# johannesu/stereo

Hardware: AMD Instinct MI355X
Metric: TRW-S fusion iterations/sec, 450x375x60 labels (higher is better)
Workload: dtype f64

## Files before the change

stereo_amd/csrc/trws_spec.h:

```cpp
#pragma once
#include <hip/hip_runtime.h>

#include <cstdint>

#include "trws_dev.h"

namespace stereo {
namespace {

constexpr int kSwConsP = 13, kSwPubP = 16, kSwFree = 18, kSwLabel = 20, kSwNode = 22, kSwKinds = 24, kSwPubM = 32;
constexpr int kRsNt = 0, kRsKinds = 1, kRsNmsg = 2, kRsCut = 5, kRsPubKinds = 6, kRsNout = 7, kRsNin = 8, kRsSrc = 9, kRsMd = 13,
              kRsNode = 14, kRsTag = 15;

typedef __attribute__((address_space(3))) int spec_lds_int;
__device__ __forceinline__ int lds_load(const int *w) { return __hip_atomic_load((const spec_lds_int *)w, __ATOMIC_RELAXED, __HIP_MEMORY_SCOPE_WORKGROUP); }
__device__ __forceinline__ void lds_store(int *w, int v) { __hip_atomic_store((spec_lds_int *)w, v, __ATOMIC_RELAXED, __HIP_MEMORY_SCOPE_WORKGROUP); }
#define SPEC_ACQUIRE() __builtin_amdgcn_fence(__ATOMIC_ACQUIRE, "workgroup", "local")
#define SPEC_RELEASE() __builtin_amdgcn_fence(__ATOMIC_RELEASE, "workgroup", "local")

template <int MASK>
__device__ __forceinline__ bool spec_keep_waiting(int &spins, long long &t0, int *abort_word, int32_t *abort_flag, long long spin_ticks) {
  spins = (spins + 1) & MASK;
  if (spins != 0) return true;
  if (lds_load(abort_word) || ld_sc1(abort_flag)) return false;
  const long long now = (long long)wall_clock64();
  if (t0 == 0) { t0 = now | 1; return true; }
  if (now - t0 > 4 * spin_ticks) { lds_store(abort_word, 1); return false; }
  return true;
}
template <bool SLEEP>
__device__ __forceinline__ bool run_wait_i(const int *word, int want, int *abort_word, int32_t *abort_flag, long long spin_ticks) {
  int spins = 0;
  long long t0 = 0;
  while (lds_load(word) < want) {
    if (SLEEP) __builtin_amdgcn_s_sleep(1);
    if (!spec_keep_waiting<SLEEP ? 1023 : 4095>(spins, t0, abort_word, abort_flag, spin_ticks)) return false;
  }
  SPEC_ACQUIRE();
  return true;
}
__device__ __attribute__((noinline)) bool run_wait(const int *word, int want, int *abort_word, int32_t *abort_flag, long long spin_ticks) {
  return run_wait_i<true>(word, want, abort_word, abort_flag, spin_ticks);
}
template <int N>
__device__ __forceinline__ bool run_wait_n(const int *words, int want, int *abort_word, int32_t *abort_flag, long long spin_ticks) {
  static_assert(N == 1 || N == 4, "run_wait_n");
  if (N == 1) return run_wait_i<true>(words, want, abort_word, abort_flag, spin_ticks);
  typedef int spec_v4i __attribute__((ext_vector_type(4)));
  typedef __attribute__((address_space(3))) const volatile spec_v4i spec_lds_v4i;
  int spins = 0;
  long long t0 = 0;
  for (;;) {
    const spec_v4i v = *(spec_lds_v4i *)words;
    if (min(min(v.x, v.y), min(v.z, v.w)) >= want) break;
    if (!spec_keep_waiting<4095>(spins, t0, abort_word, abort_flag, spin_ticks)) return false;
  }
  SPEC_ACQUIRE();
  return true;
}

template <class T>
__device__ __forceinline__ T uniform_value(T v) {
  static_assert(sizeof(T) == 4 || sizeof(T) == 8, "uniform_value");
  if (sizeof(T) == 4) {
    int w;
    __builtin_memcpy(&w, &v, 4);
    w = __builtin_amdgcn_readfirstlane(w);
    __builtin_memcpy(&v, &w, 4);
  } else {
    int w[2];
    __builtin_memcpy(w, &v, 8);
    w[0] = __builtin_amdgcn_readfirstlane(w[0]); w[1] = __builtin_amdgcn_readfirstlane(w[1]);
    __builtin_memcpy(&v, w, 8);
  }
  return v;
}
__device__ __forceinline__ DevParams uniform_params(const DevParams *pp) {
  DevParams q;
#define U(f) q.f = uniform_value(pp->f)
  U(K); U(lambda); U(unary); U(msg); U(pos); U(alpha); U(x); U(done); U(abort_flag); U(spin_ticks); U(n_own); U(N);
  U(desc[0]); U(desc[1]); U(window); U(uniform_step); U(spec_c0[0]); U(spec_c0[1]); U(spec_c1[0]); U(spec_c1[1]);
  U(spec_len); U(spec_nseg); U(spec_max_len); U(spec_rows); U(spec_x); U(spec_undo); U(spec_stat); U(timeline); U(tl_stride); U(debug);
#undef U
  return q;
}

template <int D>
__device__ __forceinline__ int draw_first_ticket(const DevParams &p, int *word) {
  if (threadIdx.x == 0) *word = next_run<D>(p);
  __syncthreads();
  const int run = __builtin_amdgcn_readfirstlane(*word);
  __syncthreads();
  return run;
}

template <class RL, bool PRIMAL, bool UPDATE>
__device__ __attribute__((noinline)) void run_publisher(const DevParams *pp_, int epoch_) {
  extern __shared__ __attribute__((aligned(16))) double spec_lds[];
  const DevParams p = uniform_params(pp_);
  constexpr int R = RL::C * kWave;
  double *rb = spec_lds + RL::kBase;
  int *abort_word = (int *)spec_lds + RL::kAbortInt;
  const int lane = threadIdx.x & (kWave - 1);
  const int epoch = __builtin_amdgcn_readfirstlane(epoch_);
  const int K = p.K;
  int *rw = (int *)(rb + RL::kWords);
  for (int s = 1; s < p.spec_nseg; ++s) {
    const int ps = s & 1;
    if (UPDATE) {
      if (!run_wait_n<RL::C>(rw + kSwPubM + 4 * ps, s, abort_word, p.abort_flag, p.spin_ticks)) return;
      const double *pb = rb + RL::kPub + ps * 2 * R;
      const int kinds = lds_load(rw + kSwKinds + ps);
#pragma unroll
      for (int c = 0; c < RL::C; ++c) {
        const int kk = c * kWave + lane;
        if (kk < K) {
          double a0 = pb[kk], a1 = pb[R + kk];
          if ((p.debug & 16384) && s % 3 == 1 && kk == 0) a0 = __longlong_as_double(__double_as_longlong(a0) ^ 1ll);
          if ((p.debug & 65536) && s % 3 == 1 && (kk & 1)) a0 += 0.375;
#pragma unroll
          for (int k = 0; k < 8; ++k) {
            const int kd = (kinds >> (4 * k)) & 15;
            if (kd) st_sc1(p.spec_rows + ((size_t)s * 8 + k) * K + kk, kd == 8 ? a0 : a1);
          }
        }
      }
    }
    if (PRIMAL) {
      if (!run_wait_i<true>(rw + kSwPubP + ps, s, abort_word, p.abort_flag, p.spin_ticks)) return;
      int label = lds_load(rw + kSwLabel + ps);
      if ((p.debug & 32768) && s % 5 == 2) label = label > 0 ? label - 1 : (K > 1 ? 1 : 0);
      if (lane == 0) st_sc1(p.spec_x + s, label);
    }
    asm volatile("s_waitcnt vmcnt(0)" ::: "memory");
    if (lane == 0) { st_sc1(p.done + p.N + s, epoch); lds_store(rw + kSwFree, s); }
  }
}

template <int C, int WAVES, int VERDICT, bool BACKWARD, bool PRIMAL, bool UPDATE>
__device__ __attribute__((noinline)) int spec_commit(const DevParams *pp_, int epoch_, int p0_, int p1_, int seg_, int compare_, int ctl_off_) {
  extern __shared__ __attribute__((aligned(16))) double spec_lds[];
  const DevParams &p = *pp_;
  const int epoch = epoch_, p0 = p0_, p1 = p1_, seg = seg_, compare = compare_;
  constexpr int D = BACKWARD ? 1 : 0;
  constexpr int DW = TrwsGraph::kDescWords;
  const int32_t *desc = p.desc[D];
  int *ctl = (int *)spec_lds + ctl_off_;
  const int tid = threadIdx.x, lane = tid & (kWave - 1);
  const int wave = __builtin_amdgcn_readfirstlane(tid / kWave);
  const int K = p.K;
  if (compare) {
    if (wave == 0) {
      int differ = 0;
      if (!wait_flag(p, p.N + p.spec_nseg + seg, epoch, -2)) { if (lane == 0) ctl[1] = 1; }
      else {
        const int w = desc[(size_t)p0 * DW + lane];
        const int f = __builtin_amdgcn_readlane(w, 2);
        const int nout = f & 15, ntot = nout + ((f >> 4) & 15);
        for (int j = nout; j < ntot; ++j) {
          if (__builtin_amdgcn_readlane(w, 12 + j) < 0) continue;
          if (UPDATE) {
            const size_t ea = ((size_t)seg * 8 + j) * K, eb = (size_t)__builtin_amdgcn_readlane(w, 4 + j) * K;
            for (int c = 0; c < C; ++c) {
              const int kk = c * kWave + lane, kc = kk < K ? kk : K - 1;
              const double a = ld_sc1(p.spec_rows + ea + kc), b = ld_sc1(p.msg + eb + kc);
              differ |= UNI(__double_as_longlong(a) != __double_as_longlong(b)) ? 1 : 0;
            }
          }
          if (PRIMAL) differ |= ld_sc1(p.spec_x + seg) != ld_sc1(p.x + __builtin_amdgcn_readlane(w, 32 + j)) ? 1 : 0;
        }
      }
      if (lane == 0) ctl[VERDICT] = differ;
    }
    __syncthreads();
    const int differ = __builtin_amdgcn_readfirstlane(ctl[VERDICT]);
    const int gave_up = __builtin_amdgcn_readfirstlane(ctl[1]);
    __syncthreads();
    if (tid == 0) ctl[VERDICT] = 0;
    if (gave_up) { if (tid == 0) st_sc1(p.abort_flag, 1); return 2; }
    if (differ) {
      if (UPDATE) {
        for (int pos = p0 + wave; pos < p1; pos += WAVES) {
          const int w = desc[(size_t)pos * DW + lane];
          const int nout = __builtin_amdgcn_readlane(w, 2) & 15;
          for (int j = 0; j < nout && j < 4; ++j) {
            const size_t em = (size_t)__builtin_amdgcn_readlane(w, 4 + j) * K, eu = ((size_t)(seg * p.spec_max_len + (pos - p0)) * 4 + j) * K;
            for (int c = 0; c < C; ++c) {
              const int kk = c * kWave + lane;
              if (kk < K) st_sc1(p.msg + em + kk, ld_sc1(p.spec_undo + eu + kk));
            }
          }
        }
        asm volatile("s_waitcnt vmcnt(0)" ::: "memory");
        __builtin_amdgcn_fence(__ATOMIC_ACQ_REL, "agent");
      }
      if (tid == 0) { ctl[3] = 1; if (p.spec_stat) atomicAdd(p.spec_stat, 1ull); }
      __syncthreads();
      return 1;
    }
  }
  if (wave == 0) {
    if (seg + 1 < p.spec_nseg && lane == 0) st_sc1(p.done + p.N + p.spec_nseg + seg + 1, epoch);
    for (int pos = p0 + lane; pos < p1; pos += kWave) st_sc1(p.done + desc[(size_t)pos * DW + 1], epoch);
    if (lane == 0 && p.spec_stat) atomicAdd(p.spec_stat + 1, 1ull);
  }
  return 0;
}

template <class RL, bool BACKWARD, bool PRIMAL, bool UPDATE>
__device__ __attribute__((noinline)) void chain_runner(const DevParams *pp_, int epoch_) {
  extern __shared__ __attribute__((aligned(16))) double spec_lds[];
  const DevParams &p = *pp_;
  const int epoch = epoch_;
  constexpr int R = RL::C * kWave, M = RL::kMsgWaves, D = BACKWARD ? 1 : 0;
  double *rb = spec_lds + RL::kBase;
  const int tid = threadIdx.x;
  const int wave = __builtin_amdgcn_readfirstlane(tid / kWave);
  const int c0 = p.spec_c0[D], c1 = p.spec_c1[D];
  int *rw = (int *)(rb + RL::kWords);
  if (tid < 64) rw[tid] = 0;
  if (tid < RL::kSlots) ((int *)(rb + tid * RL::kSlotDoubles + RL::kSc))[kRsTag] = 0;
  if (tid < 32 * RL::kTabs) {
    const int t = tid >> 5, e = tid & 31;
    rb[RL::kTab + t * (R + 32) + (e < 16 ? e : R + e)] = __builtin_huge_val();
  }
  RL::prepare(p, rb, tid);
  if (p.timeline && tid == 0) p.timeline[((size_t)2 * p.tl_stride + D) * 2] = wall_clock64();
  __syncthreads();
  const unsigned long long trole0 = wall_clock64();
  if (wave < M) { if (UPDATE) { __builtin_amdgcn_s_setprio(3); RL::template messages<BACKWARD>(pp_, wave); __builtin_amdgcn_s_setprio(0); } }
  else if (wave == M) { if (PRIMAL) { __builtin_amdgcn_s_setprio(3); RL::template labels<BACKWARD>(pp_); __builtin_amdgcn_s_setprio(0); } }
  else if (wave < M + 1 + RL::kLoaders) RL::template loader<BACKWARD, PRIMAL, UPDATE>(pp_, epoch, wave - M - 1);
  else if (wave == M + 1 + RL::kLoaders) run_publisher<RL, PRIMAL, UPDATE>(pp_, epoch);
  if (p.timeline && p.spec_stat && (tid & (kWave - 1)) == 0 && (wave == 0 || wave == M || wave == M + RL::kLoaders || wave == M + 1 + RL::kLoaders))
    p.spec_stat[8 + 4 * D + (wave == 0 ? 0 : wave == M ? 1 : wave == M + RL::kLoaders ? 2 : 3)] = wall_clock64() - trole0;
  __syncthreads();
  if (RL::kOverlay && lds_load((int *)spec_lds + RL::kAbortInt) && tid == 0) st_sc1(p.abort_flag, 1);
  if (p.timeline && tid == 0) p.timeline[((size_t)2 * p.tl_stride + D) * 2 + 1] = wall_clock64();
  if (p.spec_stat && tid == 0) atomicAdd(p.spec_stat + 2, (unsigned long long)(c1 - c0));
  if (RL::kOverlay) __syncthreads();
}

constexpr int kRunSlots = 10;
constexpr int kRunLoaders = 8;
constexpr int kRunRowP = 0, kRunRowS = 64, kRunRowM = 256, kRunRowTH = 384, kRunRowOUT = 448, kRunSc = 704;
constexpr int kRunSlotDoubles = kRunSc + 16;
constexpr int kRunTab = kRunSlots * kRunSlotDoubles;
constexpr int kRunPub = kRunTab + 96;
constexpr int kRunWords = kRunPub + 256;
constexpr int kRunDoubles = kRunWords + 32;
constexpr int kRunDummy = 32;
constexpr int kRwConsM = 12;
constexpr int kRunBase = kPipeLdsDoubles, kRunAbortInt = 2 * kPipeCtlOff + 1;

#define RLI(v, i) __builtin_amdgcn_readlane((v), (i))

struct RunNodeM {
  int sw;
  double sd, P, S0, S1, S2, M0, M1;
};
__device__ __forceinline__ void run_request_m(const double *sl, int lane, RunNodeM &n) {
  n.sw = ((const int *)(sl + kRunSc))[lane & 15];
  asm volatile("" ::: "memory");
  n.sd = sl[kRunSc + 8 + (lane & 7)];
  n.P = sl[kRunRowP + lane]; n.S0 = sl[kRunRowS + lane]; n.S1 = sl[kRunRowS + 64 + lane]; n.S2 = sl[kRunRowS + 128 + lane];
  n.M0 = sl[kRunRowM + lane]; n.M1 = sl[kRunRowM + 64 + lane];
}
struct RunArgsM {
  int K, window, c0, c1;
  double lambda, step;
  int32_t *abort_flag;
  long long spin_ticks;
  unsigned long long *stat;
};

template <bool BACKWARD, int G>
__device__ __forceinline__ bool run_visit_m(const RunArgsM &a, double *rb, int *rw, double *tabl, int *cons_word, int lane, bool act, int i, int &slot_off,
                                            RunNodeM &cur, RunNodeM &nxt, double &A0, double &A1, double (&ad)[4 * G], double &alpha_have,
                                            int *abort_word) {
  const double inf = __builtin_huge_val();
  if (__builtin_amdgcn_readlane(cur.sw, kRsTag) != i + 1) {
    const long long t0_ = (long long)wall_clock64();
    if (!__builtin_amdgcn_readfirstlane((int)run_wait((const int *)(rb + slot_off + kRunSc) + kRsTag, i + 1, abort_word, a.abort_flag, a.spin_ticks))) return false;
    run_request_m(rb + slot_off, lane, cur);
    if (a.stat && lane == 0) { atomicAdd(a.stat + 3 + 2 * (BACKWARD ? 1 : 0), 1ull); atomicAdd(a.stat + 4 + 2 * (BACKWARD ? 1 : 0), (unsigned long long)((long long)wall_clock64() - t0_)); }
  }
  const int sw = cur.sw;
  const int key = __builtin_amdgcn_readlane(sw, kRsKinds), nmsg = __builtin_amdgcn_readlane(sw, kRsNmsg), cut = __builtin_amdgcn_readlane(sw, kRsCut);
  double Di = cur.P;
  if (key == 0x20098) { Di += A0; Di += A1; }
  else if (key == 0x30908) { Di += A0; Di += cur.S0; Di += A1; }
  else if (key == 0x30098) { Di += A0; Di += A1; Di += cur.S0; }
  else if (key == 0x41908) { Di += A0; Di += cur.S0; Di += A1; Di += cur.S1; }
  else {
    const int nt = key >> 16;
    for (int t = 0; t < nt; ++t) {
      const int kd = (key >> (4 * t)) & 15;
      if (kd == 8) Di += A0; else if (kd == 9) Di += A1; else if (kd == 0) Di += cur.S0; else if (kd == 1) Di += cur.S1; else Di += cur.S2;
    }
  }
  if (BACKWARD) Di -= wave_min_dpp(act ? Di : inf);
  const double sd = cur.sd, mold0 = cur.M0, mold1 = cur.M1;
  const double gamma = readlane_f64(sd, 2);
  lds_store(cons_word, i + 1 - a.c0);
  slot_off += kRunSlotDoubles;
  if (slot_off == kRunSlots * kRunSlotDoubles) slot_off = 0;
  if (i + 1 < a.c1) run_request_m(rb + slot_off, lane, nxt);
  double R0 = 0, R1 = 0;
  for (int m = 0; m < nmsg; ++m) {
    const double alpha = readlane_f64(sd, m);
    const double h = gamma * Di - (m == 0 ? mold0 : mold1);
    double out = 0;
    if (alpha != 0) {
      *tabl = h;
      if (__builtin_expect(alpha != alpha_have, 0)) {
        asm volatile("" ::: "memory");
#pragma unroll
        for (int d = 0; d < 4 * G; ++d) ad[d] = alpha * ((double)(d + 1) * a.step);
        alpha_have = alpha;
      }
      const double hmin = wave_min_dpp(h);
      const double vtrunc = hmin + alpha * a.lambda;
      __builtin_amdgcn_fence(__ATOMIC_RELEASE, "wavefront");
      __builtin_amdgcn_wave_barrier();
      double lo[4 * G], hi[4 * G];
#pragma unroll
      for (int d = 0; d < 4 * G; ++d) { lo[d] = tabl[-(d + 1)]; hi[d] = tabl[d + 1]; }
      double ma = h, mb = vtrunc;
#pragma unroll
      for (int d = 0; d < 4 * G; ++d) { ma = min_raw(ma, lo[d] + ad[d]); mb = min_raw(mb, hi[d] + ad[d]); }
      __builtin_amdgcn_fence(__ATOMIC_ACQUIRE, "wavefront");
      __builtin_amdgcn_wave_barrier();
      out = min_raw(ma, mb) - hmin;
    }
    if (m == 0) R0 = out; else R1 = out;
  }
  A0 = R0; A1 = nmsg == 2 ? R1 : R0;
  if (cut) {
    const int ps = cut & 1;
    if (__builtin_amdgcn_readfirstlane(lds_load(rw + kSwFree)) < cut - 2 &&
        !__builtin_amdgcn_readfirstlane((int)run_wait(rw + kSwFree, cut - 2, abort_word, a.abort_flag, a.spin_ticks))) return false;
    double *pb = rb + kRunPub + ps * 128;
    pb[lane] = A0; pb[64 + lane] = A1;
    if (lane == 0) lds_store(rw + kSwKinds + ps, __builtin_amdgcn_readlane(sw, kRsPubKinds));
    SPEC_RELEASE();
    if (lane == 0) lds_store(rw + kSwPubM + 4 * ps, cut);
  }
  return true;
}

template <bool BACKWARD, int G>
__device__ __forceinline__ void run_messages_g(const RunArgsM &a, double *rb, int lane, int *abort_word) {
  const bool act = lane < a.K;
  int *rw = (int *)(rb + kRunWords);
  double *tabl = rb + kRunTab + 16 + lane;
  int *cons_word = lane == 0 ? rw + kRwConsM : (int *)(rb + kRunDoubles) + lane;
  double ad[4 * G];
#pragma unroll
  for (int d = 0; d < 4 * G; ++d) ad[d] = 0;
  double alpha_have = 0;
  double A0 = 0, A1 = 0;
  RunNodeM na, nb;
  run_request_m(rb, lane, na);
  nb = na;
  int slot_off = 0;
  for (int i = a.c0; i < a.c1; i += 2) {
    if (!run_visit_m<BACKWARD, G>(a, rb, rw, tabl, cons_word, lane, act, i, slot_off, na, nb, A0, A1, ad, alpha_have, abort_word)) return;
    if (i + 1 < a.c1 && !run_visit_m<BACKWARD, G>(a, rb, rw, tabl, cons_word, lane, act, i + 1, slot_off, nb, na, A0, A1, ad, alpha_have, abort_word)) return;
  }
}

template <bool BACKWARD>
__device__ __attribute__((noinline)) void run_messages(const DevParams *pp) {
  extern __shared__ __attribute__((aligned(16))) double run_lds[];
  constexpr int D = BACKWARD ? 1 : 0;
  RunArgsM a;
  a.K = uniform_value(pp->K); a.window = uniform_value(pp->window); a.c0 = uniform_value(pp->spec_c0[D]); a.c1 = uniform_value(pp->spec_c1[D]);
  a.lambda = uniform_value(pp->lambda); a.step = uniform_value(pp->uniform_step);
  a.abort_flag = uniform_value(pp->abort_flag); a.spin_ticks = uniform_value(pp->spin_ticks); a.stat = uniform_value(pp->spec_stat);
  double *rb = run_lds + kRunBase;
  int *abort_word = (int *)run_lds + kRunAbortInt;
  const int lane = threadIdx.x & (kWave - 1);
  if (a.window <= 4) run_messages_g<BACKWARD, 1>(a, rb, lane, abort_word);
  else run_messages_g<BACKWARD, 2>(a, rb, lane, abort_word);
}

struct RunNodeP {
  int sw;
  double sd, TH, O0, O1, O2, O3;
};
__device__ __forceinline__ void run_request_p(const double *sl, int lane, RunNodeP &n) {
  n.sw = ((const int *)(sl + kRunSc))[lane & 15];
  asm volatile("" ::: "memory");
  n.sd = sl[kRunSc + 8 + (lane & 7)];
  n.TH = sl[kRunRowTH + lane];
  n.O0 = sl[kRunRowOUT + lane]; n.O1 = sl[kRunRowOUT + 64 + lane]; n.O2 = sl[kRunRowOUT + 128 + lane]; n.O3 = sl[kRunRowOUT + 192 + lane];
}
template <bool BACKWARD>
__device__ __attribute__((noinline)) void run_labels(const DevParams *pp_) {
  extern __shared__ __attribute__((aligned(16))) double run_lds[];
  const DevParams p = uniform_params(pp_);
  double *rb = run_lds + kRunBase;
  int *abort_word = (int *)run_lds + kRunAbortInt;
  const int lane = threadIdx.x & (kWave - 1);
  const int c0 = p.spec_c0[BACKWARD ? 1 : 0], c1 = p.spec_c1[BACKWARD ? 1 : 0];
  const double inf = __builtin_huge_val();
  const int K = p.K;
  const bool act = lane < K;
  int *rw = (int *)(rb + kRunWords);
  const double posk = act ? p.pos[lane] : 0.0;
  const double lambda = p.lambda;
  int xprev = 0;
  RunNodeP cur, nxt;
  run_request_p(rb, lane, cur);
  nxt = cur;
  for (int i = c0; i < c1; ++i) {
    const double *sl = rb + ((i - c0) % kRunSlots) * kRunSlotDoubles;
    if (RLI(cur.sw, kRsTag) != i + 1) {
      if (!run_wait_i<true>((const int *)(sl + kRunSc) + kRsTag, i + 1, abort_word, p.abort_flag, p.spin_ticks)) return;
      run_request_p(sl, lane, cur);
    }
    const int sw = cur.sw;
    const double sd = cur.sd;
    const int nout = RLI(sw, kRsNout), nin = RLI(sw, kRsNin), md = RLI(sw, kRsMd), cut = RLI(sw, kRsCut);
    double db = act ? cur.TH : 0.0;
    const double o0 = cur.O0, o1 = cur.O1, o2 = cur.O2, o3 = cur.O3;
    if (lane == 0) lds_store(rw + kSwConsP, i + 1 - c0);
    if (i + 1 < c1) run_request_p(rb + ((i + 1 - c0) % kRunSlots) * kRunSlotDoubles, lane, nxt);
#pragma unroll
    for (int k = 0; k < 4; ++k) {
      if (k < nin) {
        const int src = RLI(sw, kRsSrc + k);
        const int ks = src < 0 ? xprev : src;
        const double pks = readlane_f64(posk, ks);
        const double d = ((md >> k) & 1) == 0 ? pks - posk : posk - pks;
        db += readlane_f64(sd, 3 + k) * min_raw(fabs(d), lambda);
      }
    }
    double di = db;
    if (nout > 0) di += o0;
    if (nout > 1) di += o1;
    if (nout > 2) di += o2;
    if (nout > 3) di += o3;
    const double dim = act ? di : inf;
    const double vbest = wave_min_dpp(dim);
    xprev = __builtin_ctzll(__builtin_amdgcn_ballot_w64(dim == vbest));
    if (cut) {
      const int ps = cut & 1;
      if (!run_wait_i<true>(rw + kSwFree, cut - 2, abort_word, p.abort_flag, p.spin_ticks)) return;
      if (lane == 0) { rw[kSwLabel + ps] = xprev; rw[kSwNode + ps] = RLI(sw, kRsNode); }
      SPEC_RELEASE();
      if (lane == 0) lds_store(rw + kSwPubP + ps, cut);
    }
    cur = nxt;
  }
}

template <bool BACKWARD, bool PRIMAL, bool UPDATE>
__device__ __attribute__((noinline)) void run_loader(const DevParams *pp_, int epoch_, int lw_) {
  extern __shared__ __attribute__((aligned(16))) double run_lds[];
  const DevParams p = uniform_params(pp_);
  double *rb = run_lds + kRunBase;
  int *abort_word = (int *)run_lds + kRunAbortInt;
  const int lane = threadIdx.x & (kWave - 1);
  const int epoch = __builtin_amdgcn_readfirstlane(epoch_), lw = __builtin_amdgcn_readfirstlane(lw_);
  constexpr int D = BACKWARD ? 1 : 0;
  const int c0 = p.spec_c0[D], c1 = p.spec_c1[D];
  constexpr int DW = TrwsGraph::kDescWords;
  const int32_t *desc = p.desc[D];
  const int K = p.K;
  const int lk = lane < K ? lane : K - 1;
  int *rw = (int *)(rb + kRunWords);
  const int L = p.spec_len, nseg = p.spec_nseg;
  int w2 = 0, wn2 = 0;
  if (c0 + lw < c1) { w2 = desc[(size_t)(c0 + lw) * DW + lane]; wn2 = c0 + lw + 1 < c1 ? desc[(size_t)(c0 + lw + 1) * DW + lane] : 0; }
  for (int i = c0 + lw; i < c1; i += kRunLoaders) {
    const int w = w2, wn = wn2;
    if (i + kRunLoaders < c1) {
      w2 = desc[(size_t)(i + kRunLoaders) * DW + lane];
      wn2 = i + kRunLoaders + 1 < c1 ? desc[(size_t)(i + kRunLoaders + 1) * DW + lane] : 0;
    }
    const int f = RLI(w, 2), fn = RLI(wn, 2);
    const int nout = f & 15, nin = (f >> 4) & 15, ndep = (f >> 8) & 15, md = (f >> 16) & 255, ntot = nout + nin;
    const int noutn = fn & 15, ntotn = noutn + ((fn >> 4) & 15);
    const int j8 = lane & 7;
    const int slw = __shfl(w, 12 + j8, kWave), sln = __shfl(wn, 12 + j8, kWave);
    const int fr = i > c0 ? (int)(__builtin_amdgcn_ballot_w64(lane < 8 && lane >= nout && lane < ntot && slw >= 0) & 255ull) : 0;
    const int frn = i + 1 < c1 ? (int)(__builtin_amdgcn_ballot_w64(lane < 8 && lane >= noutn && lane < ntotn && sln >= 0) & 255ull) : 0;
    const int kfirst = fr ? __builtin_ctz(fr) : ntot;
    int s0 = -1, s1 = -1;
    {
      int rest = frn;
      while (rest) {
        const int k = __builtin_ctz(rest);
        rest &= rest - 1;
        const int s = __builtin_amdgcn_readlane(wn, 12 + k);
        if (s0 < 0 || s0 == s) s0 = s; else s1 = s;
      }
    }
    int p0s = -1;
    if (fr) p0s = __builtin_amdgcn_readlane(w, 12 + kfirst);
    int kinds = 0, nt = 0, nstaged = 0, stage_of[4] = {-1, -1, -1, -1};
    for (int k = kfirst; k < ntot; ++k) {
      int kd;
      if ((fr >> k) & 1) kd = __builtin_amdgcn_readlane(w, 12 + k) == p0s ? 8 : 9;
      else { kd = nstaged; if (nstaged < 4) stage_of[nstaged] = k; ++nstaged; }
      kinds |= kd << (4 * nt);
      ++nt;
    }
    int cut = 0, pubkinds = 0;
    if (i + 1 < c1 && (i + 1 - c0) % L == 0 && (i + 1 - c0) / L < nseg) {
      cut = (i + 1 - c0) / L;
      for (int k = noutn; k < ntotn; ++k)
        if ((frn >> k) & 1) pubkinds |= (__builtin_amdgcn_readlane(wn, 12 + k) == s0 ? 8 : 9) << (4 * k);
    }
    const int fm = RLI(w, kDescFetch) & 255;
    const double *ua = p.unary + (size_t)((unsigned long long)(unsigned)RLI(w, 0) * (unsigned long long)(unsigned)K) + lk;
    const double theta = *ua;
    const double av = p.alpha[__shfl(w, 4 + j8, kWave)];
    double r[8];
#pragma unroll
    for (int k = 0; k < 8; ++k) {
      r[k] = 0;
      if (k < nout) r[k] = *(p.msg + (size_t)((unsigned long long)(unsigned)RLI(w, 4 + k) * (unsigned long long)(unsigned)K) + lk);
    }
    if (ndep > 0) wait_for_dependencies_w(p, ndep, __shfl(w, 20 + (lane & 3), kWave), RLI(w, 1), epoch, lane, abort_word);
    if (lds_load(abort_word)) return;
    int src = -1;
#pragma unroll
    for (int k = 0; k < 8; ++k) {
      if (k >= nout && k < ntot && ((fm >> k) & 1) && !((fr >> k) & 1)) {
        if (UPDATE) r[k] = ld_sc1(p.msg + (size_t)((unsigned long long)(unsigned)RLI(w, 4 + k) * (unsigned long long)(unsigned)K) + lk);
        if (PRIMAL) { const int xv = ld_sc1(p.x + RLI(w, 32 + k)); if (lane == k - nout) src = xv; }
      }
    }
    double *sl = rb + ((i - c0) % kRunSlots) * kRunSlotDoubles;
    if (UPDATE && !run_wait_i<true>(rw + kRwConsM, i - c0 - kRunSlots + 1, abort_word, p.abort_flag, p.spin_ticks)) return;
    if (PRIMAL && !run_wait_i<true>(rw + kSwConsP, i - c0 - kRunSlots + 1, abort_word, p.abort_flag, p.spin_ticks)) return;
    if (UPDATE) {
      double P = theta;
#pragma unroll
      for (int k = 0; k < 8; ++k)
        if (k < kfirst) P += r[k];
      sl[kRunRowP + lane] = P;
#pragma unroll
      for (int k = 0; k < 8; ++k) {
        if (stage_of[0] == k) sl[kRunRowS + lane] = r[k];
        if (stage_of[1] == k) sl[kRunRowS + 64 + lane] = r[k];
        if (stage_of[2] == k) sl[kRunRowS + 128 + lane] = r[k];
      }
#pragma unroll
      for (int k = 0; k < 4; ++k) {
        if (s0 == k) sl[kRunRowM + lane] = lane < K ? r[k] : -__builtin_huge_val();
        if (s1 == k) sl[kRunRowM + 64 + lane] = lane < K ? r[k] : -__builtin_huge_val();
      }
    }
    if (PRIMAL) {
      sl[kRunRowTH + lane] = theta;
#pragma unroll
      for (int k = 0; k < 4; ++k)
        if (k < nout) sl[kRunRowOUT + k * 64 + lane] = r[k];
    }
    int nmsg = s0 < 0 ? 0 : 1;
    if (UPDATE && s1 >= 0) {
      bool same = RLI(__double2hiint(av), s0) == RLI(__double2hiint(av), s1) && RLI(__double2loint(av), s0) == RLI(__double2loint(av), s1);
#pragma unroll
      for (int a = 0; a < 4; ++a)
#pragma unroll
        for (int b = 0; b < 4; ++b)
          if (a != b && s0 == a && s1 == b) same = same && !UNI(lane < K && __double_as_longlong(r[a]) != __double_as_longlong(r[b]));
      nmsg = same ? 1 : 2;
    }
    {
      int word = 0;
      word = lane == kRsNt ? nt : lane == kRsKinds ? (kinds | (nt << 16)) : lane == kRsNmsg ? nmsg : lane == kRsCut ? cut
           : lane == kRsPubKinds ? pubkinds : lane == kRsNout ? nout : lane == kRsNin ? nin : lane == kRsMd ? (md >> nout) : lane == kRsNode ? RLI(w, 0) : 0;
      const int srck = __shfl(src, lane - kRsSrc, kWave);
      if (lane >= kRsSrc && lane < kRsSrc + 4) word = srck;
      if (lane < kRsTag) ((int *)(sl + kRunSc))[lane] = word;
      const double a0 = readlane_f64(av, s0 < 0 ? 0 : s0), a1 = readlane_f64(av, s1 < 0 ? (s0 < 0 ? 0 : s0) : s1);
      const double ain = __shfl(av, nout + (lane - 3 < 0 ? 0 : lane - 3), kWave);
      const double g = (double)1 / (double)(nout > nin ? nout : nin > 0 ? nin : 1);
      if (lane < 8) sl[kRunSc + 8 + lane] = lane == 0 ? a0 : lane == 1 ? a1 : lane == 2 ? g : ain;
    }
    SPEC_RELEASE();
    if (lane == 0) lds_store((int *)(sl + kRunSc) + kRsTag, i + 1);
  }
}

struct PipeRunner {
  static constexpr int C = 1, kBase = kRunBase, kAbortInt = kRunAbortInt, kSlots = kRunSlots, kSlotDoubles = kRunSlotDoubles,
                       kSc = kRunSc, kTab = kRunTab, kTabs = 1, kPub = kRunPub, kWords = kRunWords, kMsgWaves = 1, kLoaders = kRunLoaders;
  static constexpr bool kOverlay = false;
  static __device__ __forceinline__ void prepare(const DevParams &, double *, int) {}
  template <bool BACKWARD>
  static __device__ __forceinline__ void messages(const DevParams *pp, int) { run_messages<BACKWARD>(pp); }
  template <bool BACKWARD>
  static __device__ __forceinline__ void labels(const DevParams *pp) { run_labels<BACKWARD>(pp); }
  template <bool BACKWARD, bool PRIMAL, bool UPDATE>
  static __device__ __forceinline__ void loader(const DevParams *pp, int epoch, int lw) { run_loader<BACKWARD, PRIMAL, UPDATE>(pp, epoch, lw); }
};

#undef RLI

}
}
```

Before: 129.1.

## Restructure label wave loop and reschedule message min-convolution in speculative TRW-S

The label-decoding wave is rewritten to match the message wave: a 2-way unrolled ping-pong node pipeline with an incrementally advanced slot offset instead of a modulo, per-lane consumption words, and a fast-path check before waiting on the free word. The message wave gains fast paths for the dominant per-direction kind keys and hoists alpha*lambda into a cached value. The wave min reduction is moved after the neighbour table loads, separated by scheduling barriers, so LDS latency overlaps the DPP reduction. LDS base pointers are pinned to 32-bit scalar address-space values so the compiler can use cheaper addressing. The risk is added ordering subtlety from the extra acquire fence and the changed reduction order.

```diff
diff --git a/stereo_amd/csrc/trws_spec.h b/stereo_amd/csrc/trws_spec.h
--- a/stereo_amd/csrc/trws_spec.h
+++ b/stereo_amd/csrc/trws_spec.h
@@ -15,6 +15,12 @@
 typedef __attribute__((address_space(3))) int spec_lds_int;
 __device__ __forceinline__ int lds_load(const int *w) { return __hip_atomic_load((const spec_lds_int *)w, __ATOMIC_RELAXED, __HIP_MEMORY_SCOPE_WORKGROUP); }
 __device__ __forceinline__ void lds_store(int *w, int v) { __hip_atomic_store((spec_lds_int *)w, v, __ATOMIC_RELAXED, __HIP_MEMORY_SCOPE_WORKGROUP); }
+typedef __attribute__((address_space(3))) double spec_lds_double;
+__device__ __forceinline__ double *pinned_lds(double *dyn) {
+  unsigned off = (unsigned)(size_t)(spec_lds_double *)dyn;
+  asm volatile("" : "+s"(off));
+  return (double *)(spec_lds_double *)(size_t)off;
+}
 #define SPEC_ACQUIRE() __builtin_amdgcn_fence(__ATOMIC_ACQUIRE, "workgroup", "local")
 #define SPEC_RELEASE() __builtin_amdgcn_fence(__ATOMIC_RELEASE, "workgroup", "local")
 
@@ -276,7 +282,7 @@
 
 template <bool BACKWARD, int G>
 __device__ __forceinline__ bool run_visit_m(const RunArgsM &a, double *rb, int *rw, double *tabl, int *cons_word, int lane, bool act, int i, int &slot_off,
-                                            RunNodeM &cur, RunNodeM &nxt, double &A0, double &A1, double (&ad)[4 * G], double &alpha_have,
+                                            RunNodeM &cur, RunNodeM &nxt, double &A0, double &A1, double (&ad)[4 * G], double &alpha_have, double &al,
                                             int *abort_word) {
   const double inf = __builtin_huge_val();
   if (__builtin_amdgcn_readlane(cur.sw, kRsTag) != i + 1) {
@@ -288,7 +294,13 @@
   const int sw = cur.sw;
   const int key = __builtin_amdgcn_readlane(sw, kRsKinds), nmsg = __builtin_amdgcn_readlane(sw, kRsNmsg), cut = __builtin_amdgcn_readlane(sw, kRsCut);
   double Di = cur.P;
-  if (key == 0x20098) { Di += A0; Di += A1; }
+  int key_first = key;
+  asm volatile("" : "+s"(key_first));
+  const bool between = BACKWARD && key_first == 0x30908;
+  if (BACKWARD) key_first ^= between ? 0x30908 ^ 0x30098 : 0;
+  if (!BACKWARD && __builtin_expect(key_first == 0x20098, 1)) { Di += A0; Di += A1; }
+  else if (BACKWARD && __builtin_expect(key_first == 0x30098, 1)) { Di += A0; Di += between ? cur.S0 : A1; Di += between ? A1 : cur.S0; }
+  else if (key == 0x20098) { Di += A0; Di += A1; }
   else if (key == 0x30908) { Di += A0; Di += cur.S0; Di += A1; }
   else if (key == 0x30098) { Di += A0; Di += A1; Di += cur.S0; }
   else if (key == 0x41908) { Di += A0; Di += cur.S0; Di += A1; Di += cur.S1; }
@@ -317,21 +329,24 @@
         asm volatile("" ::: "memory");
 #pragma unroll
         for (int d = 0; d < 4 * G; ++d) ad[d] = alpha * ((double)(d + 1) * a.step);
+        al = alpha * a.lambda;
         alpha_have = alpha;
       }
-      const double hmin = wave_min_dpp(h);
-      const double vtrunc = hmin + alpha * a.lambda;
       __builtin_amdgcn_fence(__ATOMIC_RELEASE, "wavefront");
       __builtin_amdgcn_wave_barrier();
       double lo[4 * G], hi[4 * G];
 #pragma unroll
       for (int d = 0; d < 4 * G; ++d) { lo[d] = tabl[-(d + 1)]; hi[d] = tabl[d + 1]; }
-      double ma = h, mb = vtrunc;
-#pragma unroll
-      for (int d = 0; d < 4 * G; ++d) { ma = min_raw(ma, lo[d] + ad[d]); mb = min_raw(mb, hi[d] + ad[d]); }
+      __builtin_amdgcn_sched_barrier(0);
+      const double hmin = wave_min_dpp(h);
+      __builtin_amdgcn_sched_barrier(0);
+      const double vtrunc = hmin + al;
+      double ma = h, mb = hi[0] + ad[0];
+#pragma unroll
+      for (int d = 0; d < 4 * G; ++d) { ma = min_raw(ma, lo[d] + ad[d]); if (d > 0) mb = min_raw(mb, hi[d] + ad[d]); }
       __builtin_amdgcn_fence(__ATOMIC_ACQUIRE, "wavefront");
       __builtin_amdgcn_wave_barrier();
-      out = min_raw(ma, mb) - hmin;
+      out = min_raw(min_raw(ma, mb), vtrunc) - hmin;
     }
     if (m == 0) R0 = out; else R1 = out;
   }
@@ -359,14 +374,15 @@
 #pragma unroll
   for (int d = 0; d < 4 * G; ++d) ad[d] = 0;
   double alpha_have = 0;
+  double al = 0;
   double A0 = 0, A1 = 0;
   RunNodeM na, nb;
   run_request_m(rb, lane, na);
   nb = na;
   int slot_off = 0;
   for (int i = a.c0; i < a.c1; i += 2) {
-    if (!run_visit_m<BACKWARD, G>(a, rb, rw, tabl, cons_word, lane, act, i, slot_off, na, nb, A0, A1, ad, alpha_have, abort_word)) return;
-    if (i + 1 < a.c1 && !run_visit_m<BACKWARD, G>(a, rb, rw, tabl, cons_word, lane, act, i + 1, slot_off, nb, na, A0, A1, ad, alpha_have, abort_word)) return;
+    if (!run_visit_m<BACKWARD, G>(a, rb, rw, tabl, cons_word, lane, act, i, slot_off, na, nb, A0, A1, ad, alpha_have, al, abort_word)) return;
+    if (i + 1 < a.c1 && !run_visit_m<BACKWARD, G>(a, rb, rw, tabl, cons_word, lane, act, i + 1, slot_off, nb, na, A0, A1, ad, alpha_have, al, abort_word)) return;
   }
 }
 
@@ -378,8 +394,9 @@
   a.K = uniform_value(pp->K); a.window = uniform_value(pp->window); a.c0 = uniform_value(pp->spec_c0[D]); a.c1 = uniform_value(pp->spec_c1[D]);
   a.lambda = uniform_value(pp->lambda); a.step = uniform_value(pp->uniform_step);
   a.abort_flag = uniform_value(pp->abort_flag); a.spin_ticks = uniform_value(pp->spin_ticks); a.stat = uniform_value(pp->spec_stat);
-  double *rb = run_lds + kRunBase;
-  int *abort_word = (int *)run_lds + kRunAbortInt;
+  double *lds0 = pinned_lds(run_lds);
+  double *rb = lds0 + kRunBase;
+  int *abort_word = (int *)lds0 + kRunAbortInt;
   const int lane = threadIdx.x & (kWave - 1);
   if (a.window <= 4) run_messages_g<BACKWARD, 1>(a, rb, lane, abort_word);
   else run_messages_g<BACKWARD, 2>(a, rb, lane, abort_word);
@@ -396,63 +413,82 @@
   n.TH = sl[kRunRowTH + lane];
   n.O0 = sl[kRunRowOUT + lane]; n.O1 = sl[kRunRowOUT + 64 + lane]; n.O2 = sl[kRunRowOUT + 128 + lane]; n.O3 = sl[kRunRowOUT + 192 + lane];
 }
+struct RunArgsP {
+  int c0, c1;
+  double lambda;
+  int32_t *abort_flag;
+  long long spin_ticks;
+};
+__device__ __forceinline__ bool run_visit_p(const RunArgsP &a, double *rb, int *rw, int *cons_word, int lane, bool act, double posk, int i, int &slot_off,
+                                            RunNodeP &cur, RunNodeP &nxt, int &xprev, int *abort_word) {
+  const double inf = __builtin_huge_val();
+  if (RLI(cur.sw, kRsTag) != i + 1) {
+    if (!__builtin_amdgcn_readfirstlane((int)run_wait((const int *)(rb + slot_off + kRunSc) + kRsTag, i + 1, abort_word, a.abort_flag, a.spin_ticks))) return false;
+    run_request_p(rb + slot_off, lane, cur);
+  }
+  const int sw = cur.sw;
+  const double sd = cur.sd;
+  const int nout = RLI(sw, kRsNout), nin = RLI(sw, kRsNin), md = RLI(sw, kRsMd), cut = RLI(sw, kRsCut);
+  double db = act ? cur.TH : 0.0;
+  const double o0 = cur.O0, o1 = cur.O1, o2 = cur.O2, o3 = cur.O3;
+  lds_store(cons_word, i + 1 - a.c0);
+  slot_off += kRunSlotDoubles;
+  if (slot_off == kRunSlots * kRunSlotDoubles) slot_off = 0;
+  if (i + 1 < a.c1) run_request_p(rb + slot_off, lane, nxt);
+#pragma unroll
+  for (int k = 0; k < 4; ++k) {
+    if (k < nin) {
+      const int src = RLI(sw, kRsSrc + k);
+      const int ks = src < 0 ? xprev : src;
+      const double pks = readlane_f64(posk, ks);
+      const double d = ((md >> k) & 1) == 0 ? pks - posk : posk - pks;
+      db += readlane_f64(sd, 3 + k) * min_raw(fabs(d), a.lambda);
+    }
+  }
+  double di = db;
+  if (nout > 0) di += o0;
+  if (nout > 1) di += o1;
+  if (nout > 2) di += o2;
+  if (nout > 3) di += o3;
+  const double dim = act ? di : inf;
+  const double vbest = wave_min_dpp(dim);
+  xprev = __builtin_ctzll(__builtin_amdgcn_ballot_w64(dim == vbest));
+  if (cut) {
+    const int ps = cut & 1;
+    if (__builtin_amdgcn_readfirstlane(lds_load(rw + kSwFree)) < cut - 2 &&
+        !__builtin_amdgcn_readfirstlane((int)run_wait(rw + kSwFree, cut - 2, abort_word, a.abort_flag, a.spin_ticks))) return false;
+    SPEC_ACQUIRE();
+    if (lane == 0) { rw[kSwLabel + ps] = xprev; rw[kSwNode + ps] = RLI(sw, kRsNode); }
+    SPEC_RELEASE();
+    if (lane == 0) lds_store(rw + kSwPubP + ps, cut);
+  }
+  return true;
+}
 template <bool BACKWARD>
-__device__ __attribute__((noinline)) void run_labels(const DevParams *pp_) {
+__device__ __attribute__((noinline)) void run_labels(const DevParams *pp) {
   extern __shared__ __attribute__((aligned(16))) double run_lds[];
-  const DevParams p = uniform_params(pp_);
-  double *rb = run_lds + kRunBase;
-  int *abort_word = (int *)run_lds + kRunAbortInt;
+  constexpr int D = BACKWARD ? 1 : 0;
+  RunArgsP a;
+  a.c0 = uniform_value(pp->spec_c0[D]); a.c1 = uniform_value(pp->spec_c1[D]); a.lambda = uniform_value(pp->lambda);
+  a.abort_flag = uniform_value(pp->abort_flag); a.spin_ticks = uniform_value(pp->spin_ticks);
+  const int K = uniform_value(pp->K);
+  const double *pos = uniform_value(pp->pos);
+  double *lds0 = pinned_lds(run_lds);
+  double *rb = lds0 + kRunBase;
+  int *abort_word = (int *)lds0 + kRunAbortInt;
   const int lane = threadIdx.x & (kWave - 1);
-  const int c0 = p.spec_c0[BACKWARD ? 1 : 0], c1 = p.spec_c1[BACKWARD ? 1 : 0];
-  const double inf = __builtin_huge_val();
-  const int K = p.K;
   const bool act = lane < K;
   int *rw = (int *)(rb + kRunWords);
-  const double posk = act ? p.pos[lane] : 0.0;
-  const double lambda = p.lambda;
+  int *cons_word = lane == 0 ? rw + kSwConsP : (int *)(rb + kRunDoubles) + lane;
+  const double posk = act ? pos[lane] : 0.0;
   int xprev = 0;
-  RunNodeP cur, nxt;
-  run_request_p(rb, lane, cur);
-  nxt = cur;
-  for (int i = c0; i < c1; ++i) {
-    const double *sl = rb + ((i - c0) % kRunSlots) * kRunSlotDoubles;
-    if (RLI(cur.sw, kRsTag) != i + 1) {
-      if (!run_wait_i<true>((const int *)(sl + kRunSc) + kRsTag, i + 1, abort_word, p.abort_flag, p.spin_ticks)) return;
-      run_request_p(sl, lane, cur);
-    }
-    const int sw = cur.sw;
-    const double sd = cur.sd;
-    const int nout = RLI(sw, kRsNout), nin = RLI(sw, kRsNin), md = RLI(sw, kRsMd), cut = RLI(sw, kRsCut);
-    double db = act ? cur.TH : 0.0;
-    const double o0 = cur.O0, o1 = cur.O1, o2 = cur.O2, o3 = cur.O3;
-    if (lane == 0) lds_store(rw + kSwConsP, i + 1 - c0);
-    if (i + 1 < c1) run_request_p(rb + ((i + 1 - c0) % kRunSlots) * kRunSlotDoubles, lane, nxt);
-#pragma unroll
-    for (int k = 0; k < 4; ++k) {
-      if (k < nin) {
-        const int src = RLI(sw, kRsSrc + k);
-        const int ks = src < 0 ? xprev : src;
-        const double pks = readlane_f64(posk, ks);
-        const double d = ((md >> k) & 1) == 0 ? pks - posk : posk - pks;
-        db += readlane_f64(sd, 3 + k) * min_raw(fabs(d), lambda);
-      }
-    }
-    double di = db;
-    if (nout > 0) di += o0;
-    if (nout > 1) di += o1;
-    if (nout > 2) di += o2;
-    if (nout > 3) di += o3;
-    const double dim = act ? di : inf;
-    const double vbest = wave_min_dpp(dim);
-    xprev = __builtin_ctzll(__builtin_amdgcn_ballot_w64(dim == vbest));
-    if (cut) {
-      const int ps = cut & 1;
-      if (!run_wait_i<true>(rw + kSwFree, cut - 2, abort_word, p.abort_flag, p.spin_ticks)) return;
-      if (lane == 0) { rw[kSwLabel + ps] = xprev; rw[kSwNode + ps] = RLI(sw, kRsNode); }
-      SPEC_RELEASE();
-      if (lane == 0) lds_store(rw + kSwPubP + ps, cut);
-    }
-    cur = nxt;
+  RunNodeP na, nb;
+  run_request_p(rb, lane, na);
+  nb = na;
+  int slot_off = 0;
+  for (int i = a.c0; i < a.c1; i += 2) {
+    if (!run_visit_p(a, rb, rw, cons_word, lane, act, posk, i, slot_off, na, nb, xprev, abort_word)) return;
+    if (i + 1 < a.c1 && !run_visit_p(a, rb, rw, cons_word, lane, act, posk, i + 1, slot_off, nb, na, xprev, abort_word)) return;
   }
 }
 
@@ -460,8 +496,9 @@
 __device__ __attribute__((noinline)) void run_loader(const DevParams *pp_, int epoch_, int lw_) {
   extern __shared__ __attribute__((aligned(16))) double run_lds[];
   const DevParams p = uniform_params(pp_);
-  double *rb = run_lds + kRunBase;
-  int *abort_word = (int *)run_lds + kRunAbortInt;
+  double *lds0 = pinned_lds(run_lds);
+  double *rb = lds0 + kRunBase;
+  int *abort_word = (int *)lds0 + kRunAbortInt;
   const int lane = threadIdx.x & (kWave - 1);
   const int epoch = __builtin_amdgcn_readfirstlane(epoch_), lw = __builtin_amdgcn_readfirstlane(lw_);
   constexpr int D = BACKWARD ? 1 : 0;
```

Measured after the change: 131.9, median of 6. 1.02x the previous value.
